# pityka/lamp

Measured on AMD Instinct MI355X. Metric: training-step samples/sec, higher is better.
Workload: dtype bf16; 1 GPU; example-cifar100 Cnn.resnet(100) training step (fwd+backprop+AdamW), synthetic CIFAR batch; per_gpu_batch=2048, global_batch=2048, parallelism=single, optimizer=AdamW lr 1e-3 wd 0 beta2 0.95 mixedPrecision

## Files before the change

### lamp_amd/_capi.py

```python
from __future__ import annotations

import ctypes as C
import os
import re

_HERE = os.path.dirname(os.path.abspath(__file__))
ROOT = os.path.dirname(_HERE)
HEADERS = [os.path.join(ROOT, "include", "lamp_hip.h"), os.path.join(ROOT, "include", "lamp_host.h")]
LIB_PATH = os.environ.get("LAMP_LIB_PATH") or os.path.join(_HERE, "lib", "liblamp_hip.so")


class LampError(RuntimeError):
    pass


_PTR = C.c_void_p
_TYPE_MAP = [
    (r"^const char\*$", C.c_char_p),
    (r"^char\*$", C.c_char_p),
    (r"^(const )?(lamp_\w+)\*\*$", C.POINTER(_PTR)),
    (r"^(const )?(lamp_\w+)\* ?const\*$", C.POINTER(_PTR)),
    (r"^(const )?(lamp_\w+)\*\[\d*\]$", C.POINTER(_PTR)),
    (r"^(const )?(lamp_\w+)\*$", _PTR),
    (r"^const uint8_t\[\d*\]$", C.POINTER(C.c_uint8)),
    (r"^(const )?uint8_t\*$", C.POINTER(C.c_uint8)),
    (r"^(const )?int64_t\*$", C.POINTER(C.c_int64)),
    (r"^(const )?double\*$", C.POINTER(C.c_double)),
    (r"^(const )?int\*$", C.POINTER(C.c_int)),
    (r"^(const )?uint64_t\*$", C.POINTER(C.c_uint64)),
    (r"^(const )?void\*\*$", C.POINTER(_PTR)),
    (r"^(const )?void\*$", _PTR),
    (r"^double$", C.c_double),
    (r"^int$", C.c_int),
    (r"^int64_t$", C.c_int64),
    (r"^uint64_t$", C.c_uint64),
    (r"^size_t$", C.c_size_t),
]


def _ctype_of(param: str):
    p = re.sub(r"/\*.*?\*/", "", param).strip()
    m = re.match(r"^(.*?)(\b\w+)?(\[\d*\])?$", p)
    arr = ""
    if "[" in p:
        arr = p[p.index("["):]
        p = p[: p.index("[")].strip()
    toks = p.replace("*", " * ").split()
    if toks and re.match(r"^\w+$", toks[-1]) and toks[-1] not in (
        "int", "double", "int64_t", "uint64_t", "size_t", "char", "void", "uint8_t", "const") and len(toks) > 1:
        toks = toks[:-1]
    t = " ".join(toks).replace(" *", "*").replace("* ", "*")
    t = re.sub(r"\s+", " ", t).strip() + arr
    t = t.replace("* const*", "* const*")
    for rx, ct in _TYPE_MAP:
        if re.match(rx, t):
            return ct
    raise LampError(f"cannot map C parameter type {param!r} (normalised {t!r})")


def parse_header(path: str):
    if not os.path.exists(path):
        return {}
    src = open(path).read()
    src = re.sub(r"/\*.*?\*/", " ", src, flags=re.S)
    src = re.sub(r"//[^\n]*", " ", src)
    src = re.sub(r"#[^\n]*", " ", src)
    decls = {}
    for m in re.finditer(r"\b(int|const char\*)\s+(lamp_\w+)\s*\(([^;{]*?)\)\s*;", src, flags=re.S):
        ret, name, params = m.group(1), m.group(2), " ".join(m.group(3).split())
        plist = [] if params in ("", "void") else [p.strip() for p in params.split(",")]
        decls[name] = (C.c_char_p if "char" in ret else C.c_int, [_ctype_of(p) for p in plist], plist)
    return decls


class _Lib:
    def __init__(self):
        self._dll = None
        self.decls = {}
        for h in HEADERS:
            self.decls.update(parse_header(h))

    def load(self):
        if self._dll is not None:
            return self._dll
        if not os.path.exists(LIB_PATH):
            raise LampError(
                f"{LIB_PATH} is missing: build it with `python -c 'import __graft_entry__ as g; g.build()'` "
                "(hipcc --offload-arch=gfx950). There is no CPU fallback.")
        os.environ.setdefault("HIP_FORCE_DEV_KERNARG", "1")
        self._dll = C.CDLL(LIB_PATH, mode=C.RTLD_LOCAL)
        self._dll.lamp_last_error.restype = C.c_char_p
        self.missing = []
        for name, (res, args, _) in self.decls.items():
            try:
                fn = getattr(self._dll, name)
            except AttributeError:
                self.missing.append(name)
                continue
            fn.restype = res
            fn.argtypes = args
        return self._dll

    def __getattr__(self, name):
        if name.startswith("_"):
            raise AttributeError(name)
        dll = self.load()
        fn = getattr(dll, name)
        if self.decls.get(name, (C.c_int,))[0] is not C.c_int:
            return fn

        def checked(*a):
            rc = fn(*a)
            if rc != 0:
                raise LampError(dll.lamp_last_error().decode("utf-8", "replace"))
            return rc

        checked.__name__ = name
        setattr(self, name, checked)
        return checked


lib = _Lib()


def i64_array(xs):
    xs = list(xs)
    return (C.c_int64 * max(len(xs), 1))(*xs)


def f64_array(xs):
    xs = list(xs)
    return (C.c_double * max(len(xs), 1))(*xs)


def handle_array(hs):
    hs = list(hs)
    return (_PTR * max(len(hs), 1))(*hs)
```

### lamp_amd/csrc/core/switches.h

```cpp
#pragma once
#include <cstdint>

namespace lamp {

constexpr int64_t SW_NO_CLAMP = INT64_MIN;

#define LAMP_SWITCHES_ONCE(X)                                                                                                             \
                                                        \
  X(conv_sibling, "LAMP_CONV_SIBLING", BOOL, 1, 0, "a residual block's 3x3 and its sibling 1x1 of the same input as one forward launch") \
  X(conv_chain, "LAMP_CONV_CHAIN", BOOL, 1, 0, "a convolution directly in front of a residual block and the block's 3x3 + 1x1 as one forward call (0: two)") \
  X(fuse_bn_pair, "LAMP_FUSE_BN_PAIR", BOOL, 1, 0, "relu(bn(right) + bn(left)) at a block's end as one op (0: the chain)")                \
  X(fuse_pool_logsoftmax, "LAMP_FUSE_POOL_LOGSOFTMAX", BOOL, 1, 0, "average pool -> flatten -> log-softmax tail as one node")             \
  X(fuse_block_tail, "LAMP_FUSE_BLOCK_TAIL", BOOL, 1, 0, "the last residual block and the pooled log-softmax tail as one node")          \
  X(fuse_bn_conv, "LAMP_FUSE_BN_CONV", BOOL, 1, 0, "batch norm -> relu -> convolution: the convolution applies the norm while staging")  \
  X(fuse_loss_accumulate, "LAMP_FUSE_LOSS_ACCUMULATE", BOOL, 1, 0, "acc += n * loss inside the NLL loss kernel")                          \
  X(fuse_loss_backward, "LAMP_FUSE_LOSS_BACKWARD", BOOL, 1, 0, "the NLL loss backward goes straight to the pooled log-softmax node's input in one launch")                      \
  X(fuse_loss_tail, "LAMP_FUSE_LOSS_TAIL", BOOL, 1, 0, "the loss launch also writes the pooled log-softmax's input gradient per plane")  \
  X(conv_dgrad_accumulate, "LAMP_CONV_DGRAD_ACCUMULATE", BOOL, 1, 0, "a convolution's input gradient adds into the existing one in its epilogue") \
  X(conv_dgrad_pair, "LAMP_CONV_DGRAD_PAIR", BOOL, 1, 0, "input gradients of a block's 3x3 and sibling 1x1 from one launch")             \
  X(conv_wgrad_pair, "LAMP_CONV_WGRAD_PAIR", BOOL, 1, 0, "weight gradients of a block's 3x3 and sibling 1x1 from one launch")            \
  X(conv_bwd_pair, "LAMP_CONV_BWD_PAIR", BOOL, 1, 0, "a block's paired input gradient and its two weight gradients from one call (0: the two pair calls)") \
  X(linear_bias_fused, "LAMP_LINEAR_BIAS_FUSED", BOOL, 1, 0, "a linear layer's bias in the GEMM epilogue (0: mm then add)")               \
  X(mult_add_fused, "LAMP_MULT_ADD_FUSED", BOOL, 1, 0, "x * scale + residual in one pass (0: mult then add)")                             \
  X(attention_as_written_for_cuda, "LAMP_ATTENTION_AS_WRITTEN_FOR_CUDA", BOOL, 0, 0, "multi-head attention as the reference's op chain instead of the fused kernels") \
  X(recurrent_fused, "LAMP_RECURRENT_FUSED", BOOL, 1, 0, "RNN / GRU / LSTM as one node per sequence with fused cell kernels (0: the fold over time steps)") \
  X(fuse_qkv, "LAMP_FUSE_QKV", BOOL, 1, 0, "self-attention's three projections as one product (0: three)")                                \
  X(host_stream_side, "LAMP_HOST_STREAM_SIDE", BOOL, 0, 0, "batch streams gather on a side stream instead of the consumer's")             \
                                                                           \
  X(pinned_cache_mb, "LAMP_PINNED_CACHE_MB", INT, 2048, 0, "upper bound of the cache of freed pinned host buffers, MiB")                  \
  X(pinned_gather_wgs, "LAMP_PINNED_GATHER_WGS", INT, 48, 1, "workgroups of a gather that reads pinned host memory")                      \
                                                                                                    \
  X(flash_attention, "LAMP_FLASH_ATTENTION", BOOL, 1, 0, "the flash attention kernels, forward and backward")                             \
  X(small_attention, "LAMP_SMALL_ATTENTION", BOOL, 1, 0, "the short-sequence attention kernels")                                          \
  X(knn_fused, "LAMP_KNN_FUSED", BOOL, 1, 0, "the fused distance + top-k nearest-neighbour kernel")                                       \
  X(knn_split, "LAMP_KNN_SPLIT", INT, -1, SW_NO_CLAMP, "f16-plane k-NN filter: 0 off, 1 where it pays, 2 forced; negative: the mode set through the API") \
  X(knn_split_planes, "LAMP_KNN_SPLIT_PLANES", INT, 0, SW_NO_CLAMP, "f16 planes per coordinate of that filter: 3, anything else 2")      \
  X(umap_pairs2, "LAMP_UMAP_PAIRS2", BOOL, 1, 0, "the UMAP loss's two-dimensional pair kernel")                                            \
                                                                                                             \
  X(gemm_shape_tags, "LAMP_GEMM_SHAPE_TAGS", BOOL, 0, 0, "profiling aid: one kernel-timer class per GEMM shape and layout")               \
  X(gemm_splitk, "LAMP_GEMM_SPLITK", BOOL, 1, 0, "split-K for products with few output tiles (bf16 and f32 / f64)")                       \
  X(gemm_tail_split, "LAMP_GEMM_TAIL_SPLIT", BOOL, 1, 0, "an almost empty last round of 256 x 256 tiles becomes a second, split-K product") \
  X(gemm_fp_split_wgs, "LAMP_GEMM_FP_SPLIT_WGS", INT, 512, 1, "workgroups an f32 / f64 split-K product aims at")                          \
                                                                                              \
  X(bn_fused_bwd, "LAMP_BN_FUSED_BWD", BOOL, 1, 0, "one-pass batch-norm backward (workgroups exchange their sums) where no mode is set through the API") \
  X(bn_fused_fp, "LAMP_BN_FUSED_FP", BOOL, 1, 0, "... its f32 / f64 form")                                                               \
  X(bn_fused_np_mask, "LAMP_BN_FUSED_NP_MASK", INT, 24, SW_NO_CLAMP, "bit mask of packets per thread (1 .. 16) at which the one-pass form runs") \
  X(bn_fused_per_cu, "LAMP_BN_FUSED_PER_CU", INT, 1, 1, "workgroups per CU the one-pass form aims at first")                              \
  X(bn_fused_small_bytes, "LAMP_BN_FUSED_SMALL_BYTES", INT, (4 << 20) + 1, SW_NO_CLAMP, "bf16 activations below this many bytes take the one-pass form whatever the mask") \
                          \
  X(conv_small2, "LAMP_CONV_SMALL2", BOOL, 1, 0, "the small-map direct convolution kernels (second generation)")                          \
  X(conv_small2_wgrad, "LAMP_CONV_SMALL2_WGRAD", BOOL, 1, 0, "... their weight gradient")                                                 \
  X(igemm_f32, "LAMP_IGEMM_F32", BOOL, 1, 0, "implicit-GEMM convolution for f32")                                                          \
  X(igemm_f64, "LAMP_IGEMM_F64", BOOL, 1, 0, "implicit-GEMM convolution for f64")                                                          \
  X(conv_bn_stats, "LAMP_CONV_BN_STATS", BOOL, 1, 0, "forward convolutions hand per-image batch-norm statistics of their output on")     \
  X(ncv_bn_stats, "LAMP_NCV_BN_STATS", BOOL, 1, 0, "... the narrow kernels' alone (needs LAMP_CONV_BN_STATS on as well)")                 \
  X(ncv_dgrad_parity, "LAMP_NCV_DGRAD_PARITY", BOOL, 1, 0, "narrow stride-2 pair input gradient: super-tiles by row parity (0: the plain form)") \
  X(ncv_pitch, "LAMP_NCV_PITCH", BOOL, 1, 0, "narrow kernels widen the LDS row pitch to a bank-conflict-free one")                        \
  X(ncv_two_shift, "LAMP_NCV_TWO_SHIFT", BOOL, 1, 0, "narrow kernels: two output phases per MFMA where the columns allow it")             \
  X(ncv_per_cu, "LAMP_NCV_PER_CU", INT, 4, 1, "narrow kernels: most workgroups per CU")                                                   \
  X(pack_cache, "LAMP_PACK_CACHE", BOOL, 1, 0, "packed filter images are cached per parameter and storage version (all four packing backends: core/pack_cache.h)") \
  X(pack_after_step, "LAMP_PACK_AFTER_STEP", BOOL, 1, 0, "the optimiser repacks every cached filter image of all four backends in place (0: lazily at first use)") \
                                                    \
  X(ig_small_d, "LAMP_IG_SMALL_D", BOOL, 1, 0, "the eight-image kernel for at most 64 output channels too")                               \
  X(ig_w8, "LAMP_IG_W8", BOOL, 1, 0, "two-image 128-row kernel: eight waves per image pair at one workgroup per CU or fewer (0: four)")  \
  X(ig_one_image, "LAMP_IG_ONE_IMAGE", BOOL, 1, 0, "... one image per workgroup at one image per CU or fewer (0: pairs)")                 \
                                                                                                 \
  X(wgrad_group, "LAMP_WGRAD_GROUP", BOOL, 1, 0, "two layers' eight-wave weight gradients parked and launched as one (0: every layer at once)") \
  X(wgrad_min_ips, "LAMP_WGRAD_MIN_IPS", INT, 0, 2, "fewest images per weight-gradient workgroup; unset (0): 2 up to 512 images, 8 above") \
  X(wg8h_dma, "LAMP_WG8H_DMA", BOOL, 1, 0, "eight-wave weight-gradient kernel: dY tiles by LDS-DMA (0: through registers, the bitwise reference of the DMA's hand-counted waits)") \
  X(defer_wgrad_reduce, "LAMP_DEFER_WGRAD_REDUCE", BOOL, 1, 0, "weight-gradient partial sums are reduced in batches, deferred until someone reads them")

#define LAMP_SWITCHES_PER_CALL(X)                                                                                                         \
  X(ig_variant, "LAMP_IG_VARIANT", LETTER, 0, 0, "bf16 implicit GEMM kernel form: b two-image 128-row, d eight-image at any batch; unset or any other letter: by geometry") \
  X(ig_ktail, "LAMP_IG_KTAIL", BOOL, 1, 0, "a 3x3's 1 .. 8 channels beyond the last whole K chunk from their own packed image (0: the padded chunk)") \
  X(knn_split_dbg, "LAMP_KNN_SPLIT_DBG", INT, 0, SW_NO_CLAMP, "3: the k-NN filter's kernel counts visits, candidates and selection cycles per wave and prints them")

using SwType_BOOL = bool;
using SwType_INT = int64_t;
using SwType_LETTER = char;
#define LAMP_SWITCH_MEMBER(member, name, kind, dflt, lo, doc) SwType_##kind member;
struct Switches { LAMP_SWITCHES_ONCE(LAMP_SWITCH_MEMBER) };
struct SwitchesNow { LAMP_SWITCHES_PER_CALL(LAMP_SWITCH_MEMBER) };
#undef LAMP_SWITCH_MEMBER

const Switches& sw();
SwitchesNow sw_now();

}
```

### lamp_amd/csrc/kernels/conv_narrow.hip

```cpp
#include "device_utils.h"
#include "conv_geom.h"
#include "conv_backends.h"
#include "../core/pack_cache.h"
#include "wgrad_reduce.h"
#include <type_traits>
#include <vector>
#include "conv_narrow_pack.h"
#include "../core/switches.h"

namespace lamp {

typedef nv_s8 __attribute__((aligned(2))) nv_s8_u;
typedef float nv_f4 __attribute__((ext_vector_type(4)));

struct NcvGeom {
  int N, C, CO;
  int H, W;
  int Hs, Ws;
  int top, left, dil;
  int Ho, Wo;
  int sh, sw, wx;
  int kh;
  int kh_inv;
  int pf;
// ... 379 lines not shown
    __syncthreads();
    NCV_STAMP_ONCE(3);
#if defined(NCV_SKIP) && (NCV_SKIP & 4)
    if (n < 0)
#endif
    if (q.pf && n + (int)gridDim.x < q.N)
      ncv_stage_load(pre, plan, src + (n + (int)gridDim.x) * img_in, src2 + (n + (int)gridDim.x) * img_in2);
    bf16_t* yc = co < co_a ? dst + ((int64_t)n * co_a + co) * HoWo : dst2 + ((int64_t)n * (q.CO - co_a) + (co - co_a)) * HoWo;
    const bf16_t* ap = ADD ? add + (int64_t)n * q.CO * HoWo + co * HoWo : nullptr;
    ncv_super_tiles<NK, SW, PH0, NS, ADD, STATS, PAR, false>(smem, q, wfr, koff, a_off, bv, co, yc, ap, sa, nullptr, 0, lane, wid, nwaves);
    if (STATS && !stats_per_wg) ncv_stats_leave<VPT>(sa, sst[it & 1], lane, wid);
    NCV_STAMP_ONCE(4);
  }
  if (STATS && it > 0) {
    if (stats_per_wg) ncv_stats_leave<VPT>(sa, sst[0], lane, wid);
    __syncthreads();
    if (stats_per_wg) ncv_stats_flush<NS>(sst[0], lane, wid, nwaves, q.CO, co_a, stats, stats2, (int)blockIdx.x, (int)gridDim.x);
    else ncv_stats_flush<NS>(sst[(it - 1) & 1], lane, wid, nwaves, q.CO, co_a, stats, stats2, (int)blockIdx.x + (it - 1) * (int)gridDim.x, q.N);
  }
#ifdef NCV_STAMP
  NCV_STAMP_AT(5);
  __builtin_amdgcn_s_waitcnt(0);
  NCV_STAMP_AT(6);
#endif
}

constexpr int NCV_CHAIN_PF = 2;
template <int NK0, int PH00, int NK1, int PH01, bool STATS>
__global__ __launch_bounds__(256, NK1 <= 5 ? 3 : 1) void ncv_chain_kernel(const bf16_t* __restrict__ x, const nv_bf8* __restrict__ wpk0, const bf16_t* __restrict__ bias0,
                                                                          bf16_t* s, NcvGeom q0, const nv_bf8* __restrict__ wpk1, const bf16_t* __restrict__ bias1,
                                                                          const bf16_t* __restrict__ bias1b, bf16_t* ya, bf16_t* yb, int co_a, NcvGeom q1,
                                                                          float* __restrict__ stats, float* __restrict__ stats2, int stats_per_wg) {
  __shared__ float sst[STATS ? 2 : 1][4][16][3];
  extern __shared__ __attribute__((aligned(16))) char smem[];
  const int img0 = q0.C * q0.Hs * q0.Ws, img1 = q1.C * q1.Hs * q1.Ws;
  unsigned short* xs0 = reinterpret_cast<unsigned short*>(smem);
  unsigned short* xs1 = xs0 + img0;
  const int tid = threadIdx.x, lane = tid & 63, wid = tid >> 6;
  const int co0 = lane & 7, co1 = lane & 15;
  const int64_t img_in = (int64_t)q0.C * q0.H * q0.W;
  NcvPreT<NCV_CHAIN_PF> pre;
  const NcvPlanT<NCV_CHAIN_PF> plan = ncv_stage_plan<NCV_CHAIN_PF>(q0, tid, 256);
  if ((int)blockIdx.x < q0.N) ncv_stage_load(pre, plan, x + blockIdx.x * img_in, x);
  nv_bf8 wfr1[NK1];
  int koff1[NK1];
  ncv_frag_setup<NK1, false>(q1, wpk1, lane, wfr1, koff1);
  const float bv0 = (bias0 && co0 < q0.CO) ? (float)bias0[co0] : 0.f;
  const float bv1 = co1 < co_a ? (bias1 ? (float)bias1[co1] : 0.f) : ((bias1b && co1 < q1.CO) ? (float)bias1b[co1 - co_a] : 0.f);
  for (int o = tid * 8; o < img0 + img1; o += 256 * 8) *reinterpret_cast<uint4*>(xs0 + o) = make_uint4(0, 0, 0, 0);
  const int ncg0 = q0.Wo / 8, ncg1 = q1.Wo / 4;
  const int a_tr0 = (lane & 15) / ncg0, a_cg0 = (lane & 15) - a_tr0 * ncg0;
  const int a_off0 = (a_tr0 * q0.sh * q0.Ws + a_cg0 * 8 + (q0.wx - PH00)) * 2;
  const int a_tr1 = (lane & 15) / ncg1, a_cg1 = (lane & 15) - a_tr1 * ncg1;
  const int a_off1 = (a_tr1 * q1.sh * q1.Ws + a_cg1 * 8 + (q1.wx - PH01)) * 2;
  const int HoWo0 = q0.Ho * q0.Wo, HoWo1 = q1.Ho * q1.Wo;
  unsigned short* mc = xs1 + (co0 * q1.Hs + q1.top) * q1.Ws + q1.left;
  constexpr int VPT = 16 * 4;
  NcvStatAcc sa{nv_f4{0.f, 0.f, 0.f, 0.f}, nv_f4{0.f, 0.f, 0.f, 0.f}, 0}, none = sa;
  int it = 0;
  for (int n = blockIdx.x; n < q0.N; n += gridDim.x, it++) {
    __syncthreads();
    if (STATS && !stats_per_wg && it > 0) ncv_stats_flush<1>(sst[(it - 1) & 1], lane, wid, 4, q1.CO, co_a, stats, stats2, n - (int)gridDim.x, q1.N);
    ncv_stage_store(xs0, pre, plan, 1);
    __syncthreads();
    if (n + (int)gridDim.x < q0.N) ncv_stage_load(pre, plan, x + (n + (int)gridDim.x) * img_in, x);
    nv_bf8 wfr0[NK0];
    int koff0[NK0];
    int lane0 = lane;
    asm volatile("" : "+v"(lane0));
    ncv_frag_setup<NK0, false>(q0, wpk0, lane0, wfr0, koff0);
    ncv_super_tiles<NK0, 1, PH00, 2, false, false, false, true>(smem, q0, wfr0, koff0, a_off0, bv0, co0, s + ((int64_t)n * q0.CO + co0) * HoWo0, nullptr, none,
                                                                mc, q1.Ws, lane, wid, 4);
    __syncthreads();
    bf16_t* yc = co1 < co_a ? ya + ((int64_t)n * co_a + co1) * HoWo1 : yb + ((int64_t)n * (q1.CO - co_a) + (co1 - co_a)) * HoWo1;
    ncv_super_tiles<NK1, 2, PH01, 1, false, STATS, false, false>(reinterpret_cast<const char*>(xs1), q1, wfr1, koff1, a_off1, bv1, co1, yc, nullptr, sa, nullptr, 0,
                                                                 lane, wid, 4);
    if (STATS && !stats_per_wg) ncv_stats_leave<VPT>(sa, sst[it & 1], lane, wid);
  }
  if (STATS && it > 0) {
    if (stats_per_wg) ncv_stats_leave<VPT>(sa, sst[0], lane, wid);
    __syncthreads();
    if (stats_per_wg) ncv_stats_flush<1>(sst[0], lane, wid, 4, q1.CO, co_a, stats, stats2, (int)blockIdx.x, (int)gridDim.x);
    else ncv_stats_flush<1>(sst[(it - 1) & 1], lane, wid, 4, q1.CO, co_a, stats, stats2, (int)blockIdx.x + (it - 1) * (int)gridDim.x, q1.N);
  }
}
#ifdef NCV_STAMP
extern "C" int lamp_debug_ncv_stamps(unsigned long long* out) { return hipMemcpyFromSymbol(out, HIP_SYMBOL(ncv_stamps), sizeof(ncv_stamps)) == hipSuccess ? 0 : 1; }
#endif

struct NcvWGeom {
  int N, Cin, Cout, H, W, Ho, Wo;
  int kh, kw, ph, pw;
  int Hs, Ws;
  int ncol;
  int IG;
  int Cout2;
};
constexpr int NCV_OFF2 = 4;

template <int NT, int SW>
__global__ __launch_bounds__(256) void ncv_wgrad_kernel(const bf16_t* __restrict__ dy, const bf16_t* __restrict__ x, float* __restrict__ partial, NcvWGeom q,
                                                        int images_per_block) {
  extern __shared__ __attribute__((aligned(16))) char smem[];
  const int tid = threadIdx.x, lane = tid & 63, wid = tid >> 6;
  const int HoWo = q.Ho * q.Wo;
  const int ximg = q.Cin * q.Hs * q.Ws * (SW == 2 ? 2 : 1);
  unsigned short* xs = reinterpret_cast<unsigned short*>(smem);
  unsigned short* ds = xs + q.IG * ximg;
  float* red = reinterpret_cast<float*>(ds + q.IG * 16 * HoWo);
  {
    const int tot = q.IG * (ximg + 16 * HoWo);
    for (int o = tid * 8; o < tot; o += 256 * 8) *reinterpret_cast<uint4*>(xs + o) = make_uint4(0, 0, 0, 0);
  }
  int coff[NT];
#pragma unroll
  for (int nt = 0; nt < NT; nt++) {
    int cidx = nt * 16 + (lane & 15);
    if (cidx >= q.ncol) cidx = 0;
    const int s = cidx % q.kw, r = (cidx / q.kw) % q.kh, ci = cidx / (q.kw * q.kh);
    if (SW == 1) coff[nt] = ((ci * q.Hs + r) * q.Ws + s - q.pw + NCV_LEFT) * 2;
    else {
      const int t = s - q.pw, par = t & 1, half = (t - par) >> 1;
      coff[nt] = (((ci * q.Hs + r) * 2 + par) * q.Ws + half + NCV_OFF2) * 2;
    }
  }
  nv_f4 acc[NT];
#pragma unroll
  for (int nt = 0; nt < NT; nt++) acc[nt] = nv_f4{0.f, 0.f, 0.f, 0.f};

  const int64_t n0 = (int64_t)blockIdx.x * images_per_block, n1 = min<int64_t>(n0 + images_per_block, q.N);
  const int chunks_per_img = HoWo >> 5;
  for (int64_t nb = n0; nb < n1; nb += q.IG) {
    const int ig = (int)min<int64_t>(q.IG, n1 - nb);
    __syncthreads();
    for (int im = 0; im < ig; im++) {
      const bf16_t* xp = x + (nb + im) * q.Cin * q.H * q.W;
      unsigned short* xi = xs + im * ximg;
      const int rc = q.W >> 3, total = q.Cin * q.H * rc;
      for (int i = tid; i < total; i += 256) {
        const int b = i % rc, a = (i / rc) % q.H, c = i / (rc * q.H);
        const uint4 v = *reinterpret_cast<const uint4*>(xp + (c * q.H + a) * q.W + b * 8);
        if (SW == 1) {
          *reinterpret_cast<uint4*>(xi + (c * q.Hs + q.ph + a) * q.Ws + NCV_LEFT + b * 8) = v;
        } else {
          uint2 ev, od;
          ev.x = (v.x & 0xffffu) | (v.y << 16); ev.y = (v.z & 0xffffu) | (v.w << 16);
          od.x = (v.x >> 16) | (v.y & 0xffff0000u); od.y = (v.z >> 16) | (v.w & 0xffff0000u);
          unsigned short* row = xi + ((c * q.Hs + q.ph + a) * 2) * q.Ws + NCV_OFF2 + b * 4;
          *reinterpret_cast<uint2*>(row) = ev;
          *reinterpret_cast<uint2*>(row + q.Ws) = od;
        }
      }
      const bf16_t* dp = dy + (nb + im) * q.Cout * HoWo;
      unsigned short* di = ds + im * 16 * HoWo;
      const int dtot = q.Cout * HoWo >> 3;
      for (int i = tid; i < dtot; i += 256) *reinterpret_cast<uint4*>(di + i * 8) = *reinterpret_cast<const uint4*>(dp + i * 8);
    }
    __syncthreads();
    const int nchunks = ig * chunks_per_img;
    for (int ch = wid; ch < nchunks; ch += 4) {
      const int pg = ch * 32 + (lane >> 4) * 8;
      const int im = pg / HoWo, pp = pg - im * HoWo;
      const int ho = pp / q.Wo, wo0 = pp - ho * q.Wo;
      const nv_s8 a = *reinterpret_cast<const nv_s8*>(ds + (im * 16 + (lane & 15)) * HoWo + pp);
      const char* xb = reinterpret_cast<const char*>(xs + im * ximg) +
                       (SW == 1 ? (ho * q.Ws + wo0) * 2 : ((ho * 2) * 2 * q.Ws + wo0) * 2);
// ... 549 lines not shown
  const NcvGeom& q = lp.q;
  const bool aligned = lp.aligned;
  const int ncg = lp.ncg, ph0 = lp.ph0, NK = lp.NK, nke = lp.nke, NS = lp.NS;
  const size_t lds = lp.lds;
  const Tensor* wsecond = sib ? sib->w : second ? second->w : nullptr;
  const NcvW wq = ncv_weights_of(w, g, dgrad, lp, wsecond, cout2);
  Hold wpk_h(ncv_packed_weights(w, wq, st, wsecond));
  const nv_bf8* wpk = reinterpret_cast<const nv_bf8*>(static_cast<const Tensor*>(wpk_h.get())->ptr<bf16_t>());
  const int lds_per_cu = ncv_lds_per_cu(lds);
  const bf16_t* bp = bias ? bias->ptr<bf16_t>() : (const bf16_t*)nullptr;
  if (aligned) {
    const int threads = lp.threads;
    if (second && !q.pf) return false;
    if (NK > 12 && !second) return false;
    const int NK2 = lp.NK2;
    const bool with_add = addend != nullptr && q.sw == 1;
    const bool bn_stats = sw().conv_bn_stats && sw().ncv_bn_stats;
    const bool with_stats = bn_stats && !dgrad && !addend && g.N >= 2 && (int64_t)q.Ho * q.Wo >= 64 && (sib || conv_stats_wanted(w->st->uid));
    const void* kfn = ncv_fwd2_fn(NK2, NS, ph0, q.sw, with_add, with_stats, nke);
    const int per_cu = std::min(lds_per_cu, kernel_occupancy(kfn, threads, lds));
    const int blocks = (int)std::min<int64_t>(g.N, (int64_t)num_cus() * per_cu);
    const double sib_fl = sib ? 2.0 * (double)g.N * cout2 * (double)g.Ho * g.Wo * (double)g.Cin : 0.0;
    const double sib_by = sib ? ((double)g.N * cout2 * g.Ho * g.Wo + (double)cout2 * g.Cin) * 2.0 : 0.0;
    const double sec_fl = second ? 2.0 * (double)g.N * cout2 * (double)g.Ho * g.Wo * (double)g.Cin : 0.0;
    const double sec_by = second ? ((double)g.N * cout2 * g.Ho * g.Wo + (double)cout2 * g.Cin) * 2.0 : 0.0;
    KernelTimer kt(dgrad ? "conv_dgrad_narrow" : "conv_fwd_narrow", conv_flops(g) + sib_fl + sec_fl, conv_bytes(g, 2) + sib_by + sec_by, st);
    const bf16_t* srcp = in->ptr<bf16_t>();
    const bf16_t* src2p = second ? second->dy->ptr<bf16_t>() : (const bf16_t*)nullptr;
    bf16_t* dstp = out->ptr<bf16_t>();
    const bf16_t* addp = with_add ? addend->ptr<bf16_t>() : (const bf16_t*)nullptr;
    if (addend_fused) *addend_fused = with_add;
    bf16_t* dst2p = sib ? sib->out->ptr<bf16_t>() : (bf16_t*)nullptr;
    const bf16_t* bias2p = (sib && sib->bias) ? sib->bias->ptr<bf16_t>() : (const bf16_t*)nullptr;
    int co_a = sib ? (int)g.Cout : q.CO;
    Hold statt, statt2;
    float* statp = nullptr;
    float* stat2p = nullptr;
    int stats_per_wg = g.N % blocks == 0 ? 1 : 0;
    const int parts = stats_per_wg ? blocks : (int)g.N;
    if (with_stats) {
      int64_t ps[1] = {(int64_t)parts * g.Cout * 3};
      statt = Hold(new_tensor(ps, 1, kF32, in->device()));
      statp = statt->ptr<float>();
      if (sib) {
        int64_t ps2[1] = {(int64_t)parts * cout2 * 3};
        statt2 = Hold(new_tensor(ps2, 1, kF32, in->device()));
        stat2p = statt2->ptr<float>();
      }
    }
    void* args[] = {(void*)&srcp, (void*)&wpk, (void*)&bp, (void*)&dstp, (void*)&q, (void*)&addp, (void*)&dst2p, (void*)&bias2p, (void*)&co_a,
                    (void*)&statp, (void*)&stat2p, (void*)&stats_per_wg, (void*)&src2p};
    HIP_CHECK(hipLaunchKernel(kfn, dim3(blocks), dim3(threads), args, lds, st));
    LAMP_LAUNCH_CHECK();
    if (statt.get()) conv_stats_publish(out, statt.get(), parts, sib ? 0 : w->st->uid);
    if (statt2.get()) conv_stats_publish(sib->out, statt2.get(), parts);
    return true;
  }
  if (NK > 12) return false;
  const int blocks = (int)std::min<int64_t>(g.N, (int64_t)num_cus() * lds_per_cu);
  KernelTimer kt(dgrad ? "conv_dgrad_narrow" : "conv_fwd_narrow", conv_flops(g), conv_bytes(g, 2), st);
  switch (NK) {
    case 1: ncv_launch<1>(in->ptr<bf16_t>(), wpk, bp, out->ptr<bf16_t>(), q, blocks, lds, st); break;
    case 2: ncv_launch<2>(in->ptr<bf16_t>(), wpk, bp, out->ptr<bf16_t>(), q, blocks, lds, st); break;
    case 4: ncv_launch<4>(in->ptr<bf16_t>(), wpk, bp, out->ptr<bf16_t>(), q, blocks, lds, st); break;
    case 5: ncv_launch<5>(in->ptr<bf16_t>(), wpk, bp, out->ptr<bf16_t>(), q, blocks, lds, st); break;
    case 6: case 8: ncv_launch<8>(in->ptr<bf16_t>(), wpk, bp, out->ptr<bf16_t>(), q, blocks, lds, st); break;
    default: ncv_launch<12>(in->ptr<bf16_t>(), wpk, bp, out->ptr<bf16_t>(), q, blocks, lds, st); break;
  }
  LAMP_LAUNCH_CHECK();
  return true;
}

bool narrow_conv_fwd(const Tensor* x, const Tensor* w, const Tensor* bias, Tensor* y, const ConvGeom& g, hipStream_t st) {
  return ncv_run(x, w, bias, y, g, false, st);
}
static bool ncv_fwd_pair_shapes(const Tensor* x, const ConvGeom& g, const ConvGeom& g1) {
  const bool on = sw().conv_sibling;
  if (!on || x->dtype != kBF16) return false;
  if (g.kh != 3 || g.kw != 3 || g.ph != 1 || g.pw != 1 || g1.kh != 1 || g1.kw != 1 || g1.ph != 0 || g1.pw != 0) return false;
  if (g.sh != g1.sh || g.sw != g1.sw || g.Ho != g1.Ho || g.Wo != g1.Wo || g.Cin != g1.Cin || g.N != g1.N || g.groups != 1 || g1.groups != 1) return false;
  if (g.dh != 1 || g.dw != 1 || g1.dh != 1 || g1.dw != 1) return false;
  return true;
}
bool narrow_conv_fwd_pair(const Tensor* x, const Tensor* w, const Tensor* bias, Tensor* y, const ConvGeom& g, const Tensor* w1, const Tensor* bias1,
                          Tensor* y1, const ConvGeom& g1, hipStream_t st) {
  if (!ncv_fwd_pair_shapes(x, g, g1)) return false;
  const NcvSibling sb{w1, bias1, y1};
  return ncv_run(x, w, bias, y, g, false, st, nullptr, nullptr, &sb);
}
bool narrow_conv_chain_pair(const Tensor* x, const Tensor* w0, const Tensor* bias0, Tensor* s, const ConvGeom& g0, const Tensor* w, const Tensor* bias,
                            Tensor* y, const ConvGeom& g, const Tensor* w1, const Tensor* bias1, Tensor* y1, const ConvGeom& g1, hipStream_t st) {
  if (!ncv_fwd_pair_shapes(x, g, g1)) return false;
  if (g0.groups != 1 || g0.sh != 1 || g0.sw != 1 || g0.N != g.N || g0.Cout != g.Cin || g0.Ho != g.H || g0.Wo != g.W) return false;
  const int cout2 = (int)w1->sizes[0];
  NcvLaunchPlan p0, p1;
  if (!ncv_plan(g0, x->dtype, false, false, false, 0, p0) || !ncv_plan(g, x->dtype, false, true, false, cout2, p1)) return false;
  if (!p0.aligned || !p1.aligned || p0.threads != 256 || p1.threads != 256) return false;
  if ((int64_t)p0.q.C * p0.q.H * p0.q.W > (int64_t)NCV_CHAIN_PF * 256 * 8) return false;
  p0.q.pf = 1;
  if (p0.NS != 2 || p0.NK2 != 4 || p0.ph0 != 6) return false;
  if (p1.NS != 1 || p1.q.sw != 2 || p1.ph0 != 7 || !(p1.NK2 == 5 || p1.NK2 == 12)) return false;
  const size_t lds = p0.lds + p1.lds;
  if (lds > 150 * 1024) return false;
  const NcvGeom& q0 = p0.q;
  const NcvGeom& q1 = p1.q;
  const bool with_stats = sw().conv_bn_stats && sw().ncv_bn_stats && g.N >= 2 && (int64_t)q1.Ho * q1.Wo >= 64;
  const void* kfn = nullptr;
  if (p1.NK2 == 5) kfn = with_stats ? (const void*)ncv_chain_kernel<4, 6, 5, 7, true> : (const void*)ncv_chain_kernel<4, 6, 5, 7, false>;
  else kfn = with_stats ? (const void*)ncv_chain_kernel<4, 6, 12, 7, true> : (const void*)ncv_chain_kernel<4, 6, 12, 7, false>;
  if (lds > 64 * 1024) allow_big_lds(kfn);
  const void* kpair = ncv_fwd2_fn(p1.NK2, 1, 7, 2, false, with_stats, 0);
  const int pair_per_cu = std::min(ncv_lds_per_cu(p1.lds), kernel_occupancy(kpair, 256, p1.lds));
  const int pair_blocks = (int)std::min<int64_t>(g.N, (int64_t)num_cus() * pair_per_cu);
  const int per_cu = std::min(pair_per_cu, std::min(ncv_lds_per_cu(lds), kernel_occupancy(kfn, 256, lds)));
  const int blocks = (int)std::min<int64_t>(g.N, (int64_t)num_cus() * per_cu);
  const bool pair_per_wg = g.N % pair_blocks == 0;
  if (with_stats && blocks != pair_blocks && pair_per_wg && g.N > pair_blocks) return false;
  int stats_per_wg = (blocks == pair_blocks && pair_per_wg) ? 1 : 0;
  const int parts = stats_per_wg ? blocks : (int)g.N;
  Hold wpk0_h(ncv_packed_weights(w0, ncv_weights_of(w0, g0, false, p0, nullptr, 0), st));
  Hold wpk1_h(ncv_packed_weights(w, ncv_weights_of(w, g, false, p1, w1, cout2), st, w1));
  const nv_bf8* wpk0 = reinterpret_cast<const nv_bf8*>(static_cast<const Tensor*>(wpk0_h.get())->ptr<bf16_t>());
  const nv_bf8* wpk1 = reinterpret_cast<const nv_bf8*>(static_cast<const Tensor*>(wpk1_h.get())->ptr<bf16_t>());
  Hold statt, statt2;
  float* statp = nullptr;
  float* stat2p = nullptr;
  if (with_stats) {
    int64_t ps[1] = {(int64_t)parts * g.Cout * 3}, ps2[1] = {(int64_t)parts * cout2 * 3};
    statt = Hold(new_tensor(ps, 1, kF32, x->device()));
    statt2 = Hold(new_tensor(ps2, 1, kF32, x->device()));
    statp = statt->ptr<float>(); stat2p = statt2->ptr<float>();
  }
  {
    const double fl = conv_flops(g0) + conv_flops(g) + 2.0 * (double)g.N * cout2 * (double)g.Ho * g.Wo * (double)g.Cin;
    const double by = conv_bytes(g0, 2) + conv_bytes(g, 2) + ((double)g.N * cout2 * g.Ho * g.Wo + (double)cout2 * g.Cin) * 2.0 -
                      (double)g.N * g.Cin * g.H * g.W * 2.0;
    KernelTimer kt("conv_fwd_narrow", fl, by, st);
    const bf16_t* xp = x->ptr<bf16_t>();
    const bf16_t* b0p = bias0 ? bias0->ptr<bf16_t>() : (const bf16_t*)nullptr;
    const bf16_t* bp = bias ? bias->ptr<bf16_t>() : (const bf16_t*)nullptr;
    const bf16_t* b1p = bias1 ? bias1->ptr<bf16_t>() : (const bf16_t*)nullptr;
    bf16_t* sp = s->ptr<bf16_t>();
    bf16_t* yp = y->ptr<bf16_t>();
    bf16_t* y1p = y1->ptr<bf16_t>();
    int co_a = (int)g.Cout;
    void* args[] = {(void*)&xp, (void*)&wpk0, (void*)&b0p, (void*)&sp, (void*)&q0, (void*)&wpk1, (void*)&bp, (void*)&b1p, (void*)&yp, (void*)&y1p,
                    (void*)&co_a, (void*)&q1, (void*)&statp, (void*)&stat2p, (void*)&stats_per_wg};
    HIP_CHECK(hipLaunchKernel(kfn, dim3(blocks), dim3(256), args, lds, st));
    LAMP_LAUNCH_CHECK();
  }
  if (statt.get()) conv_stats_publish(y, statt.get(), parts, 0);
  if (statt2.get()) conv_stats_publish(y1, statt2.get(), parts);
  return true;
}
bool narrow_conv_dgrad(const Tensor* dy, const Tensor* w, Tensor* dx, const ConvGeom& g, hipStream_t st, const Tensor* addend, bool* addend_fused) {
  return ncv_run(dy, w, nullptr, dx, g, true, st, addend, addend_fused);
}
bool narrow_conv_dgrad_pair(const Tensor* dy, const Tensor* w, const ConvGeom& g, const Tensor* dy1, const Tensor* w1, const ConvGeom& g1, Tensor* dx,
                            hipStream_t st, const Tensor* addend, bool* addend_fused) {
  if (addend_fused) *addend_fused = false;
  const bool on = sw().conv_dgrad_pair;
  if (!on || dy->dtype != kBF16 || dy1->dtype != kBF16) return false;
  if (g.kh != 3 || g.kw != 3 || g.ph != 1 || g.pw != 1 || g1.kh != 1 || g1.kw != 1 || g1.ph != 0 || g1.pw != 0) return false;
  if (g.sh != g1.sh || g.sw != g1.sw || g.Ho != g1.Ho || g.Wo != g1.Wo || g.H != g1.H || g.W != g1.W || g.Cin != g1.Cin || g.N != g1.N) return false;
  if (g.groups != 1 || g1.groups != 1 || g.dh != 1 || g.dw != 1 || g1.dh != 1 || g1.dw != 1 || g1.Cout > 16) return false;
  const NcvSecondGrad sg{dy1, w1};
  return ncv_run(dy, w, nullptr, dx, g, true, st, addend, addend_fused, nullptr, &sg);
}

// ... 234 lines not shown
```

Baseline: 2.265 million samples/s.

## Fuse stride-2 3x3 and sibling 1x1 conv with separate wave roles

Adds a forward kernel in which half of the waves compute a narrow stride-2 3x3 convolution and the other half compute its sibling 1x1 from the same staged input tile in shared memory. It is used when the two convolutions together have more than 16 output channels, where the existing sibling path does not apply, so the input is loaded once and one launch replaces two. It falls back when occupancy or block counts differ from the separate kernels. The Python loader also calls lamp_has_gpu once at library load.

```diff
diff --git a/lamp_amd/_capi.py b/lamp_amd/_capi.py
--- a/lamp_amd/_capi.py
+++ b/lamp_amd/_capi.py
@@ -99,6 +99,9 @@
                 continue
             fn.restype = res
             fn.argtypes = args
+        if "lamp_has_gpu" not in self.missing:
+            n = C.c_int(0)
+            self._dll.lamp_has_gpu(C.byref(n))
         return self._dll
 
     def __getattr__(self, name):
diff --git a/lamp_amd/csrc/core/switches.h b/lamp_amd/csrc/core/switches.h
--- a/lamp_amd/csrc/core/switches.h
+++ b/lamp_amd/csrc/core/switches.h
@@ -9,6 +9,7 @@
                                                         \
   X(conv_sibling, "LAMP_CONV_SIBLING", BOOL, 1, 0, "a residual block's 3x3 and its sibling 1x1 of the same input as one forward launch") \
   X(conv_chain, "LAMP_CONV_CHAIN", BOOL, 1, 0, "a convolution directly in front of a residual block and the block's 3x3 + 1x1 as one forward call (0: two)") \
+  X(conv_pair_waves, "LAMP_CONV_PAIR_WAVES", BOOL, 1, 0, "a narrow stride-2 3x3 and its sibling 1x1 of more than 16 output channels together as one forward launch, the 1x1 on waves of its own (0: two)") \
   X(fuse_bn_pair, "LAMP_FUSE_BN_PAIR", BOOL, 1, 0, "relu(bn(right) + bn(left)) at a block's end as one op (0: the chain)")                \
   X(fuse_pool_logsoftmax, "LAMP_FUSE_POOL_LOGSOFTMAX", BOOL, 1, 0, "average pool -> flatten -> log-softmax tail as one node")             \
   X(fuse_block_tail, "LAMP_FUSE_BLOCK_TAIL", BOOL, 1, 0, "the last residual block and the pooled log-softmax tail as one node")          \
diff --git a/lamp_amd/csrc/kernels/conv_narrow.hip b/lamp_amd/csrc/kernels/conv_narrow.hip
--- a/lamp_amd/csrc/kernels/conv_narrow.hip
+++ b/lamp_amd/csrc/kernels/conv_narrow.hip
@@ -485,6 +485,57 @@
     __syncthreads();
     if (stats_per_wg) ncv_stats_flush<1>(sst[0], lane, wid, 4, q1.CO, co_a, stats, stats2, (int)blockIdx.x, (int)gridDim.x);
     else ncv_stats_flush<1>(sst[(it - 1) & 1], lane, wid, 4, q1.CO, co_a, stats, stats2, (int)blockIdx.x + (it - 1) * (int)gridDim.x, q1.N);
+  }
+}
+template <int NKA, int NKB, int SW, bool STATS>
+__global__ __launch_bounds__(256, (NKA <= 5 && NKB <= 2) ? 3 : 1) void ncv_pair_waves_kernel(const bf16_t* __restrict__ src, const nv_bf8* __restrict__ wpka, const nv_bf8* __restrict__ wpkb,
+                                                             const bf16_t* __restrict__ biasa, const bf16_t* __restrict__ biasb, bf16_t* dsta, bf16_t* dstb,
+                                                             NcvGeom qa, NcvGeom qb, float* __restrict__ statsa, float* __restrict__ statsb, int stats_per_wg) {
+  __shared__ float sst[STATS ? 2 : 1][2][2][16][3];
+  extern __shared__ __attribute__((aligned(16))) char smem[];
+  unsigned short* xs = reinterpret_cast<unsigned short*>(smem);
+  constexpr int P = 8 / SW;
+  const int tid = threadIdx.x, lane = tid & 63, nthreads = blockDim.x, w = nthreads >> 7;
+  const int role = (tid >> 6) >= w ? 1 : 0, rw = (tid >> 6) - role * w;
+  const int co = lane & 15;
+  const int64_t img_in = (int64_t)qa.C * qa.H * qa.W;
+  NcvPre pre;
+  const NcvPlan plan = ncv_stage_plan(qa, tid, nthreads);
+  if ((int)blockIdx.x < qa.N) ncv_stage_load(pre, plan, src + blockIdx.x * img_in, src);
+  nv_bf8 wfra[NKA], wfrb[NKB];
+  int koffa[NKA], koffb[NKB];
+  if (role == 0) ncv_frag_setup<NKA, false>(qa, wpka, lane, wfra, koffa);
+  else ncv_frag_setup<NKB, false>(qb, wpkb, lane, wfrb, koffb);
+  const int CO = role ? qb.CO : qa.CO;
+  const bf16_t* bias = role ? biasb : biasa;
+  bf16_t* dst = role ? dstb : dsta;
+  float* stats = role ? statsb : statsa;
+  const float bv = (bias && co < CO) ? (float)bias[co] : 0.f;
+  const int HoWo = qa.Ho * qa.Wo;
+  const int img_elems = qa.C * qa.Hs * qa.Ws;
+  for (int o = tid * 8; o < img_elems; o += nthreads * 8) *reinterpret_cast<uint4*>(xs + o) = make_uint4(0, 0, 0, 0);
+  const int ncg = qa.Wo / P;
+  const int a_tr = (lane & 15) / ncg, a_cg = (lane & 15) - a_tr * ncg;
+  const int a_off = role ? ((a_tr * qb.sh + qb.top) * qb.Ws + a_cg * 8 + qb.wx) * 2 : (a_tr * qa.sh * qa.Ws + a_cg * 8 + (qa.wx - 7)) * 2;
+  constexpr int VPT = 16 * P;
+  NcvStatAcc sa{nv_f4{0.f, 0.f, 0.f, 0.f}, nv_f4{0.f, 0.f, 0.f, 0.f}, 0};
+  int it = 0;
+  for (int n = blockIdx.x; n < qa.N; n += gridDim.x, it++) {
+    __syncthreads();
+    if (STATS && !stats_per_wg && it > 0) ncv_stats_flush<1>(sst[(it - 1) & 1][role], lane, rw, w, CO, CO, stats, nullptr, n - (int)gridDim.x, qa.N);
+    ncv_stage_store(xs, pre, plan, 1);
+    __syncthreads();
+    if (n + (int)gridDim.x < qa.N) ncv_stage_load(pre, plan, src + (n + (int)gridDim.x) * img_in, src);
+    bf16_t* yc = dst + ((int64_t)n * CO + co) * HoWo;
+    if (role == 0) ncv_super_tiles<NKA, SW, 7, 1, false, STATS, false, false>(smem, qa, wfra, koffa, a_off, bv, co, yc, nullptr, sa, nullptr, 0, lane, rw, w);
+    else ncv_super_tiles<NKB, SW, 0, 1, false, STATS, false, false>(smem, qb, wfrb, koffb, a_off, bv, co, yc, nullptr, sa, nullptr, 0, lane, rw, w);
+    if (STATS && !stats_per_wg) ncv_stats_leave<VPT>(sa, sst[it & 1][role], lane, rw);
+  }
+  if (STATS && it > 0) {
+    if (stats_per_wg) ncv_stats_leave<VPT>(sa, sst[0][role], lane, rw);
+    __syncthreads();
+    if (stats_per_wg) ncv_stats_flush<1>(sst[0][role], lane, rw, w, CO, CO, stats, nullptr, (int)blockIdx.x, (int)gridDim.x);
+    else ncv_stats_flush<1>(sst[(it - 1) & 1][role], lane, rw, w, CO, CO, stats, nullptr, (int)blockIdx.x + (it - 1) * (int)gridDim.x, qa.N);
   }
 }
 #ifdef NCV_STAMP
@@ -1200,9 +1251,76 @@
   if (g.dh != 1 || g.dw != 1 || g1.dh != 1 || g1.dw != 1) return false;
   return true;
 }
+static const void* ncv_pair_waves_fn(int nka, int nkb, bool with_stats) {
+#define NCV_PW(NKAv, NKBv) (with_stats ? (const void*)ncv_pair_waves_kernel<NKAv, NKBv, 2, true> : (const void*)ncv_pair_waves_kernel<NKAv, NKBv, 2, false>)
+#define NCV_PW_B(NKAv) (nkb == 2 ? NCV_PW(NKAv, 2) : nkb == 4 ? NCV_PW(NKAv, 4) : (const void*)nullptr)
+  const void* kfn = nka == 4 ? NCV_PW_B(4) : nka == 5 ? NCV_PW_B(5) : nka == 12 ? NCV_PW_B(12) : (const void*)nullptr;
+#undef NCV_PW_B
+#undef NCV_PW
+  return kfn;
+}
+static bool ncv_fwd_pair_waves(const Tensor* x, const Tensor* w, const Tensor* bias, Tensor* y, const ConvGeom& g, const Tensor* w1, const Tensor* bias1,
+                               Tensor* y1, const ConvGeom& g1, hipStream_t st) {
+  if (!sw().conv_pair_waves) return false;
+  if (g.N < num_cus()) return false;
+  NcvLaunchPlan pa, pb;
+  if (!ncv_plan(g, x->dtype, false, false, false, 0, pa) || !ncv_plan(g1, x->dtype, false, false, false, 0, pb)) return false;
+  if (!pa.aligned || !pb.aligned || pa.NS != 1 || pb.NS != 1) return false;
+  if (pa.q.sw != 2 || pb.q.sw != 2 || pa.ph0 != 7 || pb.ph0 != 0 || pa.ncg != pb.ncg) return false;
+  const int nsuper = pa.q.Ho / (16 / pa.ncg), wv = std::min(2, nsuper), threads = 2 * wv * 64;
+  if (pa.threads != 64 * wv || pb.threads != 64 * wv) return false;
+  if ((int64_t)pa.q.C * pa.q.H * pa.q.W > (int64_t)NCV_PF * threads * 8) return false;
+  if (pb.q.Ws > pa.q.Ws || pa.q.top + pb.q.Hs > pa.q.Hs) return false;
+  const bool with_stats = sw().conv_bn_stats && sw().ncv_bn_stats && g.N >= 2 && (int64_t)pa.q.Ho * pa.q.Wo >= 64;
+  const void* kfn = ncv_pair_waves_fn(pa.NK2, pb.NK2, with_stats);
+  if (!kfn) return false;
+  const void* ka = ncv_fwd2_fn(pa.NK2, 1, 7, 2, false, with_stats, 0);
+  const void* kb = ncv_fwd2_fn(pb.NK2, 1, 0, 2, false, with_stats, 0);
+  const int64_t cus = num_cus();
+  const int blocks_a = (int)std::min<int64_t>(g.N, cus * std::min(ncv_lds_per_cu(pa.lds), kernel_occupancy(ka, pa.threads, pa.lds)));
+  const int blocks_b = (int)std::min<int64_t>(g.N, cus * std::min(ncv_lds_per_cu(pb.lds), kernel_occupancy(kb, pb.threads, pb.lds)));
+  const int blocks = (int)std::min<int64_t>(g.N, cus * std::min(ncv_lds_per_cu(pa.lds), kernel_occupancy(kfn, threads, pa.lds)));
+  if (blocks != blocks_a || blocks != blocks_b) return false;
+  NcvGeom qa = pa.q, qb = pb.q;
+  qa.pf = 1;
+  qb.Hs = qa.Hs; qb.Ws = qa.Ws; qb.top = qa.top;
+  Hold wpka_h(ncv_packed_weights(w, ncv_weights_of(w, g, false, pa, nullptr, 0), st));
+  Hold wpkb_h(ncv_packed_weights(w1, ncv_weights_of(w1, g1, false, pb, nullptr, 0), st));
+  const nv_bf8* wpka = reinterpret_cast<const nv_bf8*>(static_cast<const Tensor*>(wpka_h.get())->ptr<bf16_t>());
+  const nv_bf8* wpkb = reinterpret_cast<const nv_bf8*>(static_cast<const Tensor*>(wpkb_h.get())->ptr<bf16_t>());
+  int stats_per_wg = g.N % blocks == 0 ? 1 : 0;
+  const int parts = stats_per_wg ? blocks : (int)g.N;
+  Hold statt, statt2;
+  float* statp = nullptr;
+  float* stat2p = nullptr;
+  if (with_stats) {
+    int64_t ps[1] = {(int64_t)parts * g.Cout * 3}, ps2[1] = {(int64_t)parts * g1.Cout * 3};
+    statt = Hold(new_tensor(ps, 1, kF32, x->device()));
+    statt2 = Hold(new_tensor(ps2, 1, kF32, x->device()));
+    statp = statt->ptr<float>(); stat2p = statt2->ptr<float>();
+  }
+  {
+    const double fl1 = 2.0 * (double)g.N * g1.Cout * (double)g.Ho * g.Wo * (double)g.Cin;
+    const double by1 = ((double)g.N * g1.Cout * g.Ho * g.Wo + (double)g1.Cout * g.Cin) * 2.0;
+    KernelTimer kt("conv_fwd_narrow", conv_flops(g) + fl1, conv_bytes(g, 2) + by1, st);
+    const bf16_t* xp = x->ptr<bf16_t>();
+    const bf16_t* bp = bias ? bias->ptr<bf16_t>() : (const bf16_t*)nullptr;
+    const bf16_t* b1p = bias1 ? bias1->ptr<bf16_t>() : (const bf16_t*)nullptr;
+    bf16_t* yp = y->ptr<bf16_t>();
+    bf16_t* y1p = y1->ptr<bf16_t>();
+    void* args[] = {(void*)&xp, (void*)&wpka, (void*)&wpkb, (void*)&bp, (void*)&b1p, (void*)&yp, (void*)&y1p, (void*)&qa, (void*)&qb,
+                    (void*)&statp, (void*)&stat2p, (void*)&stats_per_wg};
+    HIP_CHECK(hipLaunchKernel(kfn, dim3(blocks), dim3(threads), args, pa.lds, st));
+    LAMP_LAUNCH_CHECK();
+  }
+  if (statt.get()) conv_stats_publish(y, statt.get(), parts, 0);
+  if (statt2.get()) conv_stats_publish(y1, statt2.get(), parts);
+  return true;
+}
 bool narrow_conv_fwd_pair(const Tensor* x, const Tensor* w, const Tensor* bias, Tensor* y, const ConvGeom& g, const Tensor* w1, const Tensor* bias1,
                           Tensor* y1, const ConvGeom& g1, hipStream_t st) {
   if (!ncv_fwd_pair_shapes(x, g, g1)) return false;
+  if (g.Cout + g1.Cout > 16) return ncv_fwd_pair_waves(x, w, bias, y, g, w1, bias1, y1, g1, st);
   const NcvSibling sb{w1, bias1, y1};
   return ncv_run(x, w, bias, y, g, false, st, nullptr, nullptr, &sb);
 }
```

Measured after the change: 2.287 million samples/s (median of 6 runs). No clear change (+1.0%).
